# fischer-hub/panGNN

Hardware: NVIDIA B200
Metric: train_edges_per_s (higher is better)
Workload: dtype f32

## Files before the change

include/pangnn_b200.h:

```cpp
#ifndef PANGNN_B200_H
#define PANGNN_B200_H

#include <stddef.h>
#include <stdint.h>

#ifdef __cplusplus
extern "C" {
#endif

#define PANGNN_ABI_VERSION 4

#define PANGNN_OK 0
#define PANGNN_EINVAL (-1)
#define PANGNN_EWORKSPACE (-2)
#define PANGNN_ECUDA (-3)

#define PANGNN_ACT_NONE 0
#define PANGNN_ACT_ELU 1

int pangnn_abi_version(void);
const char *pangnn_last_error(void);
const char *pangnn_source_digest(void);

size_t pangnn_sort_pairs_workspace_bytes(int64_t n);
// ... 25 lines not shown
                          const float *w, const float *dis, int32_t num_nodes, int rows_are_dst,
                          float *val, void *stream);

int pangnn_gcn_aggregate(const int64_t *rowptr, const int32_t *col, const float *val, const float *x,
                         int64_t ldx, int32_t num_rows, int32_t feat, const float *bias, int act,
                         float *y, int64_t ldy, void *stream);

int pangnn_act_bwd_bias(const float *dy, const float *y, int64_t num_rows, int32_t feat, int act,
                        float *g, float *dbias , void *ws, size_t ws_bytes,
                        void *stream);
size_t pangnn_act_bwd_bias_workspace_bytes(int64_t num_rows, int32_t feat);

size_t pangnn_gemm_tn_workspace_bytes(int64_t num_rows, int32_t m, int32_t k);
int pangnn_gemm_tn(const float *a, int64_t lda, const float *b, int64_t ldb, int64_t num_rows,
                   int32_t m, int32_t k, float *c, void *ws, size_t ws_bytes, void *stream);

int pangnn_node_linear(const float *x, int64_t ldx, int64_t num_rows, int32_t k, const float *w,
                       int64_t ldw, int w_is_kn, int32_t n, const float *bias, int act, float *y,
                       int64_t ldy, void *stream);
int pangnn_node_linear_push(const float *x, int64_t ldx, int64_t num_rows, int32_t k, const float *w,
                            int64_t ldw, int w_is_kn, int32_t n, const float *bias, int act, float *y,
                            int64_t ldy, const int32_t *push_slot0, float *peer_y0, int64_t lo0, int64_t hi0,
                            const int32_t *push_slot1, float *peer_y1, int64_t lo1, int64_t hi1, void *stream);

size_t pangnn_hits_sort_unique_workspace_bytes(int64_t num_hits);
int pangnn_hits_sort_unique(const int32_t *q, const int32_t *t, const double *bits, int64_t num_hits,
                            int32_t num_nodes, int32_t *q_out, int32_t *t_out, double *bits_out,
                            uint32_t *count , void *ws, size_t ws_bytes, void *stream);
size_t pangnn_hits_normalize_workspace_bytes(int64_t num_hits);
int pangnn_hits_normalize(const int32_t *q, const int32_t *t, const double *bits, int64_t num_hits,
                          const int32_t *genome_of, const int32_t *group_of, double temp, double eps,
                          double pseudo, int drop_trivial, int32_t *src, int32_t *dst, float *w,
                          float *y, uint32_t *count , void *ws, size_t ws_bytes,
                          void *stream);

int pangnn_rows_gather_copy(const float *src, int64_t ld_src, const int32_t *idx, int64_t n, int32_t feat, float *dst,
                            int64_t ld_dst, void *stream);
int pangnn_rows_scatter_add(const float *src, int64_t ld_src, const int32_t *idx, int64_t n, int32_t feat, float *dst,
                            int64_t ld_dst, void *stream);

#define PANGNN_GRAD_REDUCE_MAX_TENSORS 32
#define PANGNN_GRAD_REDUCE_MAX_RANKS 8
int64_t pangnn_grad_bucket_floats(const int64_t *numels, int32_t count);
int pangnn_grad_push(float *const *grads, const int64_t *numels, int32_t count, float *bucket, int64_t half_floats,
                     int32_t *const *peer_signals, int32_t world, int32_t rank, int32_t *ctrl, void *stream);
int pangnn_grad_reduce(float *const *grads, const int64_t *numels, int32_t count, const float *const *peer_buckets,
// ... 123 lines not shown
```

pangnn_b200/_abi.py:

```python
import ctypes as C
import os

from . import build as _build

_c_p = C.c_void_p
_i64, _i32, _sz, _f32, _f64, _int = C.c_int64, C.c_int32, C.c_size_t, C.c_float, C.c_double, C.c_int

SIGNATURES = {
    "pangnn_abi_version": (_int, []),
    "pangnn_last_error": (C.c_char_p, []),
    "pangnn_source_digest": (C.c_char_p, []),
    "pangnn_sort_pairs_workspace_bytes": (_sz, [_i64]),
    "pangnn_sort_pairs_u64": (_int, [_c_p, _c_p, _c_p, _c_p, _i64, _int, _c_p, _sz, _c_p]),
    "pangnn_scan_workspace_bytes": (_sz, [_i64]),
    "pangnn_exclusive_scan_u32": (_int, [_c_p, _c_p, _i64, _c_p, _c_p, _sz, _c_p]),
    "pangnn_csr_build_workspace_bytes": (_sz, [_i64]),
    "pangnn_csr_build": (_int, [_c_p, _i64, _i32, _int, _c_p, _c_p, _c_p, _c_p, _sz, _c_p]),
    "pangnn_gcn_norm": (_int, [_c_p, _c_p, _c_p, _c_p, _i32, _c_p, _c_p, _c_p]),
    "pangnn_gcn_norm_apply": (_int, [_c_p, _c_p, _c_p, _c_p, _c_p, _i32, _int, _c_p, _c_p]),
    "pangnn_gcn_aggregate": (_int, [_c_p, _c_p, _c_p, _c_p, _i64, _i32, _i32, _c_p, _int, _c_p, _i64, _c_p]),
    "pangnn_act_bwd_bias": (_int, [_c_p, _c_p, _i64, _i32, _int, _c_p, _c_p, _c_p, _sz, _c_p]),
    "pangnn_act_bwd_bias_workspace_bytes": (_sz, [_i64, _i32]),
    "pangnn_gemm_tn_workspace_bytes": (_sz, [_i64, _i32, _i32]),
    "pangnn_gemm_tn": (_int, [_c_p, _i64, _c_p, _i64, _i64, _i32, _i32, _c_p, _c_p, _sz, _c_p]),
    "pangnn_node_linear": (_int, [_c_p, _i64, _i64, _i32, _c_p, _i64, _int, _i32, _c_p, _int, _c_p, _i64, _c_p]),
    "pangnn_node_linear_push": (_int, [_c_p, _i64, _i64, _i32, _c_p, _i64, _int, _i32, _c_p, _int, _c_p, _i64,
                                       _c_p, _c_p, _i64, _i64, _c_p, _c_p, _i64, _i64, _c_p]),
    "pangnn_hits_sort_unique_workspace_bytes": (_sz, [_i64]),
    "pangnn_hits_sort_unique": (_int, [_c_p, _c_p, _c_p, _i64, _i32, _c_p, _c_p, _c_p, _c_p, _c_p, _sz, _c_p]),
    "pangnn_hits_normalize_workspace_bytes": (_sz, [_i64]),
    "pangnn_hits_normalize": (_int, [_c_p, _c_p, _c_p, _i64, _c_p, _c_p, _f64, _f64, _f64, _int,
                                     _c_p, _c_p, _c_p, _c_p, _c_p, _c_p, _sz, _c_p]),
    "pangnn_rows_gather_copy": (_int, [_c_p, _i64, _c_p, _i64, _i32, _c_p, _i64, _c_p]),
    "pangnn_rows_scatter_add": (_int, [_c_p, _i64, _c_p, _i64, _i32, _c_p, _i64, _c_p]),
    "pangnn_grad_bucket_floats": (_i64, [_c_p, _i32]),
    "pangnn_grad_push": (_int, [_c_p, _c_p, _i32, _c_p, _i64, _c_p, _i32, _i32, _c_p, _c_p]),
    "pangnn_grad_reduce": (_int, [_c_p, _c_p, _i32, _c_p, _i64, _c_p, _i32, _i32, _c_p, _i64, _c_p]),
    "pangnn_edges_sorted": (_int, [_c_p, _i64, _i32, _c_p, _c_p]),
    "pangnn_csr_from_sorted": (_int, [_c_p, _i64, _i32, _c_p, _c_p, _c_p, _c_p]),
    "pangnn_csr_transpose": (_int, [_c_p, _c_p, _c_p, _i64, _i32, _c_p, _c_p, _c_p, _c_p, _sz, _c_p]),
    "pangnn_csr_merge_band": (_int, [_c_p, _c_p, _c_p, _i64, _i64, _i32, _int, _c_p, _c_p, _c_p, _c_p]),
    "pangnn_csr_spmv2": (_int, [_c_p, _c_p, _c_p, _c_p, _i32, _c_p, _c_p, _c_p]),
    "pangnn_rank1_affine_act": (_int, [_c_p, _c_p, _c_p, _c_p, _c_p, _i64, _i32, _int, _c_p, _i64, _c_p]),
    "pangnn_rank1_bwd_workspace_bytes": (_sz, [_i64, _i32]),
    "pangnn_rank1_bwd": (_int, [_c_p, _c_p, _c_p, _c_p, _i64, _i32, _int, _c_p, _c_p, _sz, _c_p]),
    "pangnn_parse_hits_tsv_workspace_bytes": (_sz, [_i64]),
    "pangnn_tsv_line_index": (_int, [_c_p, _i64, _c_p, _i64, _c_p, _c_p, _sz, _c_p]),
    "pangnn_tsv_parse_hits": (_int, [_c_p, _i64, _c_p, _i64, _i64, _i32, _c_p, _c_p, _i32, _c_p, _c_p, _c_p, _c_p]),
    "pangnn_components_init": (_int, [_c_p, _i32, _c_p]),
    "pangnn_components_round": (_int, [_c_p, _c_p, _c_p, _i64, _c_p, _i32, _c_p, _c_p]),
# ... 65 lines not shown
```

pangnn_b200/csrc/common.cuh:

```cuda
#pragma once
#include <cuda_runtime.h>
#include <stdint.h>
#include <stdio.h>

#include "../../include/pangnn_b200.h"

namespace pangnn {

constexpr int kWarp = 32;
constexpr int kNumSMs = 148;

void set_error(const char *fmt, ...);

inline int check_cuda(cudaError_t e, const char *what) {
    if (e != cudaSuccess) {
        set_error("%s: %s", what, cudaGetErrorString(e));
        return PANGNN_ECUDA;
    }
    return PANGNN_OK;
}

#define PANGNN_CHECK_LAUNCH(name)                                           \
    do {                                                                    \
        int _rc = ::pangnn::check_cuda(cudaGetLastError(), name);           \
// ... 28 lines not shown
#pragma unroll
    for (int o = 16; o > 0; o >>= 1) v += __shfl_xor_sync(0xffffffffu, v, o);
    return v;
}
__device__ __forceinline__ double warp_sum(double v) {
#pragma unroll
    for (int o = 16; o > 0; o >>= 1) v += __shfl_xor_sync(0xffffffffu, v, o);
    return v;
}
__device__ __forceinline__ double warp_max(double v) {
#pragma unroll
    for (int o = 16; o > 0; o >>= 1) v = fmax(v, __shfl_xor_sync(0xffffffffu, v, o));
    return v;
}

__device__ __forceinline__ float4 ld_stream_f4(const float *p) {
    float4 r;
    asm volatile("ld.global.nc.L1::no_allocate.v4.f32 {%0,%1,%2,%3}, [%4];"
                 : "=f"(r.x), "=f"(r.y), "=f"(r.z), "=f"(r.w)
                 : "l"(p));
    return r;
}

}
```

pangnn_b200/csrc/node_linear.cu:

```cuda
#include "common.cuh"
#include "umma.cuh"

namespace pangnn {

namespace {

constexpr int kTileM = 128;
constexpr int kKC = 32;
constexpr int kThreadsNL = 256;
constexpr int kThreadsNLAll = kThreadsNL + 32;
constexpr uint32_t kChunkA = kTileM * 16 + 16;

__device__ __forceinline__ float elu1f(float x) { return x > 0.f ? x : __expf(x) - 1.0f; }

struct NLPush {
    const int32_t *slot0, *slot1;
    float *peer0, *peer1;
    int64_t lo0, hi0, lo1, hi1;
};

template <int N, int K>
struct NLSmem {
    static constexpr uint32_t chunkB = N * 16 + 16;
    static constexpr uint32_t bytesB = (K / 4) * chunkB;
    static constexpr uint32_t bytesA = (kKC / 4) * kChunkA;
    static constexpr uint32_t ringSlot = kTileM * kKC * 4;
    static constexpr uint32_t budget = 227u * 1024u - 2048u;
    static constexpr int stages = ((int64_t)budget - (int64_t)(2 * bytesB + 4 * bytesA + 256) - 8 * 32 * (32 * 4 + 16)) / (int64_t)ringSlot >= 3 ? 2 : 1;
    static constexpr int partC = (budget - (2 * bytesB + 2 * bytesA + 256) - 8 * 32 * (32 * 4 + 16)) / ringSlot >= 3 ? 32 : 16;
    static constexpr uint32_t stageRow = partC * 4 + 16;
    static constexpr uint32_t bytesStage = 8 * 32 * stageRow;
    static constexpr uint32_t fixed = 2 * bytesB + 2 * stages * bytesA + bytesStage + 256;
    static constexpr int ringSlots = ((budget - fixed) / ringSlot) > 6 ? 6 : (int)((budget - fixed) / ringSlot);
    static constexpr uint32_t offBhi = 0, offBlo = bytesB, offA = 2 * bytesB;
    static constexpr uint32_t offStage = (offA + 2 * stages * bytesA + 127) / 128 * 128;
    static constexpr uint32_t offRing = (offStage + bytesStage + 127) / 128 * 128;
    static constexpr uint32_t total = offRing + ringSlots * ringSlot + 64;
    static constexpr int tmemCols = 4 * N;
    static_assert(ringSlots >= 2, "ring too small");
};

__device__ __forceinline__ void cp_async16(uint32_t dst_smem, const void *src) {
    asm volatile("cp.async.cg.shared.global [%0], [%1], 16;" :: "r"(dst_smem), "l"(src) : "memory");
}
__device__ __forceinline__ void cp_async_commit() { asm volatile("cp.async.commit_group;" ::: "memory"); }
template <int NPENDING>
__device__ __forceinline__ void cp_async_wait() { asm volatile("cp.async.wait_group %0;" :: "n"(NPENDING) : "memory"); }

template <int N, int K>
__global__ void __launch_bounds__(kThreadsNLAll, 1)
node_linear_kernel(const float *__restrict__ x, int64_t ldx, int64_t M, const float *__restrict__ w,
                   int64_t ldw, int w_is_kn, const float *__restrict__ bias, int act,
                   float *__restrict__ y, int64_t ldy, const NLPush push) {
    using S = NLSmem<N, K>;
    extern __shared__ __align__(128) uint8_t smem[];
    __shared__ __align__(8) uint64_t bar_stage[2], bar_ready[2], bar_full[2], bar_dfree[2];
    __shared__ uint32_t tmem_base_s;
    const int tid = threadIdx.x, warp = tid >> 5, lane = tid & 31;
    const uint32_t sbase = umma::smem_u32(smem);
    constexpr int NCH = K / kKC;
    constexpr int RS = S::ringSlots;

    if (warp == 0) umma::tmem_alloc(&tmem_base_s, S::tmemCols);
    if (tid == 32) {
        umma::mbar_init(&bar_stage[0], 1);
        umma::mbar_init(&bar_stage[1], 1);
        umma::mbar_init(&bar_full[0], 1);
        umma::mbar_init(&bar_full[1], 1);
        umma::mbar_init(&bar_ready[0], kThreadsNL);
        umma::mbar_init(&bar_ready[1], kThreadsNL);
        umma::mbar_init(&bar_dfree[0], kThreadsNL);
        umma::mbar_init(&bar_dfree[1], kThreadsNL);
        umma::fence_mbar_init();
    }
    for (int idx = tid; idx < N * K; idx += kThreadsNLAll) {
        int n, k;
// ... 12 lines not shown
    const uint32_t tmem_d = tmem_base_s;

    const int64_t num_tiles = (M + kTileM - 1) / kTileM;
    const int64_t my_tiles = blockIdx.x < num_tiles ? (num_tiles - blockIdx.x + gridDim.x - 1) / gridDim.x : 0;
    const int64_t n_items = my_tiles * NCH;
    const int f = tid & 7, rb = tid >> 3;
    constexpr uint32_t idesc = umma::idesc_tf32(kTileM, N, false, false);

    auto issue_item = [&](int64_t it) {
        if (it < n_items) {
            const int64_t tile = blockIdx.x + (it / NCH) * gridDim.x;
            const int c = (int)(it % NCH);
            const uint32_t slot = sbase + S::offRing + (uint32_t)(it % RS) * S::ringSlot;
#pragma unroll
            for (int i = 0; i < 4; ++i) {
                const int r = rb + 32 * i;
                const int64_t row = tile * kTileM + r;
                if (row < M) cp_async16(slot + (uint32_t)r * 128 + (uint32_t)f * 16, x + row * ldx + c * kKC + f * 4);
            }
        }
        cp_async_commit();
    };

    auto epilogue = [&](int64_t t_local) {
        const int64_t tile = blockIdx.x + t_local * gridDim.x;
        const int buf = (int)(t_local & 1);
        umma::mbar_wait(&bar_full[buf], (uint32_t)((t_local >> 1) & 1));
        umma::fence_after_sync();
        const int q = warp & 3, h = warp >> 2;
        constexpr int COLS = N / 2;
        constexpr int PC = S::partC;
        uint8_t *stg = smem + S::offStage + (uint32_t)warp * 32 * S::stageRow;
        const int64_t row0 = tile * kTileM + q * 32;
#pragma unroll
        for (int part = 0; part < COLS / PC; ++part) {
            const int c0 = h * COLS + part * PC;
            float v[PC], vs[PC];
            const uint32_t ta = tmem_d + (uint32_t)(buf * 2 * N) + ((uint32_t)(q * 32) << 16) + (uint32_t)c0;
            umma::tmem_ld<PC>(ta, v);
            umma::tmem_ld<PC>(ta + N, vs);
#pragma unroll
            for (int j = 0; j < PC; ++j) v[j] += vs[j];
#pragma unroll
            for (int j = 0; j < PC; j += 4) {
                float4 o = make_float4(v[j], v[j + 1], v[j + 2], v[j + 3]);
                if (bias) {
                    const float4 b = __ldg(reinterpret_cast<const float4 *>(bias + c0 + j));
                    o.x += b.x; o.y += b.y; o.z += b.z; o.w += b.w;
                }
                if (act == PANGNN_ACT_ELU) { o.x = elu1f(o.x); o.y = elu1f(o.y); o.z = elu1f(o.z); o.w = elu1f(o.w); }
                *reinterpret_cast<float4 *>(stg + (uint32_t)lane * S::stageRow + j * 4) = o;
            }
            __syncwarp();
            constexpr int LPR = PC / 4;
#pragma unroll
            for (int r0 = 0; r0 < 32; r0 += 32 / LPR) {
                const int r = r0 + lane / LPR, fl = lane % LPR;
                const float4 o = *reinterpret_cast<const float4 *>(stg + (uint32_t)r * S::stageRow + fl * 16);
                if (row0 + r < M) {
                    *reinterpret_cast<float4 *>(y + (row0 + r) * ldy + c0 + fl * 4) = o;
                    const int64_t gr = row0 + r;
                    if (push.slot0 && gr >= push.lo0 && gr < push.hi0) {
                        const int32_t ps = __ldg(push.slot0 + gr);
                        if (ps >= 0) *reinterpret_cast<float4 *>(push.peer0 + (int64_t)ps * ldy + c0 + fl * 4) = o;
                    }
                    if (push.slot1 && gr >= push.lo1 && gr < push.hi1) {
                        const int32_t ps = __ldg(push.slot1 + gr);
                        if (ps >= 0) *reinterpret_cast<float4 *>(push.peer1 + (int64_t)ps * ldy + c0 + fl * 4) = o;
                    }
                }
            }
            __syncwarp();
        }
        umma::fence_before_sync();
    };

    constexpr int ST = S::stages;
    if (warp == kThreadsNL / 32) {
#pragma unroll 1
        for (int64_t it = 0; it < n_items; ++it) {
            const int64_t t_local = it / NCH;
            const int c = (int)(it % NCH);
// ... 37 lines not shown
            if (it >= ST) umma::mbar_wait(&bar_stage[st], (uint32_t)(((it - ST) / ST) & 1));
            const uint32_t offAhi = S::offA + (uint32_t)st * 2 * S::bytesA, offAlo = offAhi + S::bytesA;
#pragma unroll
            for (int i = 0; i < 4; ++i) {
                float4 hi, lo;
                umma::split4(raw[i], hi, lo);
                const uint32_t off = (uint32_t)f * kChunkA + (uint32_t)(rb + 32 * i) * 16;
                *reinterpret_cast<float4 *>(smem + offAhi + off) = hi;
                *reinterpret_cast<float4 *>(smem + offAlo + off) = lo;
            }
            umma::fence_async_smem();
            umma::mbar_arrive(&bar_ready[st]);
            if (c == 0 && t_local > 0) {
                epilogue(t_local - 1);
                umma::mbar_arrive(&bar_dfree[(t_local - 1) & 1]);
            }
        }
        if (my_tiles > 0) epilogue(my_tiles - 1);
        cp_async_wait<0>();
    }
    umma::fence_before_sync();
    __syncthreads();
    if (warp == 0) umma::tmem_dealloc(tmem_d, S::tmemCols);
}

template <int N, int K>
int launch_node_linear(const float *x, int64_t ldx, int64_t M, const float *w, int64_t ldw, int w_is_kn,
                       const float *bias, int act, float *y, int64_t ldy, const NLPush &push, cudaStream_t st) {
    using S = NLSmem<N, K>;
    static bool attr_set = false;
    if (!attr_set) {
        int rc = check_cuda(cudaFuncSetAttribute(node_linear_kernel<N, K>, cudaFuncAttributeMaxDynamicSharedMemorySize,
                                                 (int)S::total), "cudaFuncSetAttribute(node_linear)");
        if (rc) return rc;
        attr_set = true;
    }
    const int64_t tiles = (M + kTileM - 1) / kTileM;
    const unsigned grid = (unsigned)(tiles < kNumSMs ? tiles : kNumSMs);
    node_linear_kernel<N, K><<<grid, kThreadsNLAll, S::total, st>>>(x, ldx, M, w, ldw, w_is_kn, bias, act, y, ldy, push);
    PANGNN_CHECK_LAUNCH("node_linear");
    return PANGNN_OK;
}

}
}

using namespace pangnn;

static int node_linear_dispatch(const float *x, int64_t ldx, int64_t num_rows, int32_t k, const float *w, int64_t ldw,
                                int w_is_kn, int32_t n, const float *bias, int act, float *y, int64_t ldy,
                                const NLPush &push, void *stream) {
    PANGNN_REQUIRE(num_rows >= 0, "negative row count");
    if (num_rows == 0) return PANGNN_OK;
    PANGNN_REQUIRE(x && w && y, "null pointer");
    PANGNN_REQUIRE((n == 64 || n == 128) && (k == 64 || k == 128), "n and k must be 64 or 128");
    PANGNN_REQUIRE(ldx % 4 == 0 && ldy % 4 == 0 && ldx >= k && ldy >= n, "bad row stride");
    PANGNN_REQUIRE(ldw >= (w_is_kn ? n : k), "bad weight stride");
    PANGNN_REQUIRE((uintptr_t)x % 16 == 0 && (uintptr_t)y % 16 == 0 && (!bias || (uintptr_t)bias % 16 == 0),
                   "pointers must be 16-byte aligned");
    PANGNN_REQUIRE((!push.slot0 || (push.peer0 && (uintptr_t)push.peer0 % 16 == 0)) &&
                       (!push.slot1 || (push.peer1 && (uintptr_t)push.peer1 % 16 == 0)), "bad push target");
    cudaStream_t st = (cudaStream_t)stream;
    if (n == 64 && k == 64) return launch_node_linear<64, 64>(x, ldx, num_rows, w, ldw, w_is_kn, bias, act, y, ldy, push, st);
    if (n == 128 && k == 64) return launch_node_linear<128, 64>(x, ldx, num_rows, w, ldw, w_is_kn, bias, act, y, ldy, push, st);
    if (n == 64 && k == 128) return launch_node_linear<64, 128>(x, ldx, num_rows, w, ldw, w_is_kn, bias, act, y, ldy, push, st);
    return launch_node_linear<128, 128>(x, ldx, num_rows, w, ldw, w_is_kn, bias, act, y, ldy, push, st);
}

extern "C" int pangnn_node_linear(const float *x, int64_t ldx, int64_t num_rows, int32_t k, const float *w,
                                  int64_t ldw, int w_is_kn, int32_t n, const float *bias, int act, float *y,
                                  int64_t ldy, void *stream) {
    return node_linear_dispatch(x, ldx, num_rows, k, w, ldw, w_is_kn, n, bias, act, y, ldy, NLPush{nullptr, nullptr, nullptr, nullptr, 0, 0, 0, 0},
                                stream);
}

extern "C" int pangnn_node_linear_push(const float *x, int64_t ldx, int64_t num_rows, int32_t k, const float *w,
                                       int64_t ldw, int w_is_kn, int32_t n, const float *bias, int act, float *y,
                                       int64_t ldy, const int32_t *push_slot0, float *peer_y0, int64_t lo0, int64_t hi0,
                                       const int32_t *push_slot1, float *peer_y1, int64_t lo1, int64_t hi1,
                                       void *stream) {
    return node_linear_dispatch(x, ldx, num_rows, k, w, ldw, w_is_kn, n, bias, act, y, ldy,
                                NLPush{push_slot0, push_slot1, peer_y0, peer_y1, lo0, hi0, lo1, hi1}, stream);
}
```

pangnn_b200/csrc/rank1.cu:

```cuda
#include "common.cuh"

namespace pangnn {

int reduce_partials(const float *partial, int64_t nblocks, int32_t width, int32_t stride, float *out,
                    cudaStream_t st);

__global__ void __launch_bounds__(256)
csr_spmv2_kernel(const int64_t *__restrict__ rowptr, const int32_t *__restrict__ col, const float *__restrict__ val,
                 const float *__restrict__ x, int32_t N, float *__restrict__ ax, float *__restrict__ a1) {
    const int lane = threadIdx.x & 31;
    const int64_t row = ((int64_t)blockIdx.x * blockDim.x + threadIdx.x) >> 5;
    if (row >= N) return;
    const int64_t b = rowptr[row], e = rowptr[row + 1];
    double sx = 0.0, s1 = 0.0;
    for (int64_t i = b + lane; i < e; i += 32) {
        const double v = (double)val[i];
        s1 += v;
        sx += x ? v * (double)x[col[i]] : v;
    }
    sx = warp_sum(sx);
    s1 = warp_sum(s1);
    if (lane == 0) {
        ax[row] = (float)sx;
        a1[row] = (float)s1;
    }
}

__device__ __forceinline__ float act_apply(float x, int act) {
    return (act == PANGNN_ACT_ELU && x <= 0.f) ? expm1f(x) : x;
}

__global__ void __launch_bounds__(256)
rank1_affine_act_kernel(const float *__restrict__ a, const float *__restrict__ c, const float *__restrict__ u,
                        const float *__restrict__ v, const float *__restrict__ bias, int64_t num_rows, int32_t fq,
                        int act, float *__restrict__ y, int64_t ldy) {
    const int64_t i = (int64_t)blockIdx.x * blockDim.x + threadIdx.x;
    if (i >= num_rows * fq) return;
    const int64_t r = i / fq;
    const int t = (int)(i % fq);
    const float ar = a[r], cr = c[r];
    const float4 uu = __ldg(reinterpret_cast<const float4 *>(u) + t), vv = __ldg(reinterpret_cast<const float4 *>(v) + t);
    float4 bb = make_float4(0.f, 0.f, 0.f, 0.f);
    if (bias) bb = __ldg(reinterpret_cast<const float4 *>(bias) + t);
    float4 o;
    o.x = act_apply(fmaf(ar, uu.x, fmaf(cr, vv.x, bb.x)), act);
    o.y = act_apply(fmaf(ar, uu.y, fmaf(cr, vv.y, bb.y)), act);
    o.z = act_apply(fmaf(ar, uu.z, fmaf(cr, vv.z, bb.z)), act);
    o.w = act_apply(fmaf(ar, uu.w, fmaf(cr, vv.w, bb.w)), act);
    reinterpret_cast<float4 *>(y + r * ldy)[t] = o;
}

constexpr int kR1RowsPerChunk = 64;
constexpr int kR1MaxBlocks = kNumSMs * 8;

__global__ void __launch_bounds__(256)
rank1_bwd_kernel(const float *__restrict__ dy, const float *__restrict__ yv, const float *__restrict__ a,
                 const float *__restrict__ c, int64_t num_rows, int32_t feat, int act, float *__restrict__ partial) {
    extern __shared__ float4 red[];
    const int fq = feat / 4;
    const int tx = threadIdx.x % fq, ty = threadIdx.x / fq;
    const int TY = blockDim.x / fq;
    const int64_t nchunks = (num_rows + kR1RowsPerChunk - 1) / kR1RowsPerChunk;
    float4 s0 = make_float4(0.f, 0.f, 0.f, 0.f), s1 = s0, s2 = s0;
    if (ty < TY) {
        for (int64_t chunk = blockIdx.x; chunk < nchunks; chunk += gridDim.x) {
            const int64_t r0 = chunk * kR1RowsPerChunk;
            const int64_t r1 = min(r0 + (int64_t)kR1RowsPerChunk, num_rows);
            for (int64_t r = r0 + ty; r < r1; r += TY) {
                float4 d = ld_stream_f4(dy + r * feat + tx * 4);
                if (act == PANGNN_ACT_ELU) {
                    const float4 o = ld_stream_f4(yv + r * feat + tx * 4);
// ... 91 lines not shown
```

pangnn_b200/gnn.py:

```python
import math

import torch
from torch import nn

from . import ops
from .setup import args


_SIDE_STREAMS = {}

OPERATOR_LAYER = {"kind": "function"}


def set_operator_layer(kind):
    if kind not in ("function", "library"):
        raise ValueError("operator layer is 'function' or 'library'")
    OPERATOR_LAYER["kind"] = kind


def _side_stream(device):
    key = torch.device(device).index
    if key not in _SIDE_STREAMS:
        _SIDE_STREAMS[key] = torch.cuda.Stream(device=device)
    return _SIDE_STREAMS[key]
# ... 28 lines not shown
        super().__init__()
        self.device = device
        node_embedding_dim, hidden_dim = dims
        if categorical_nodes:
            num = dataset if isinstance(dataset, int) else int(getattr(dataset, "num_genes", 0) or len(dataset.x))
            self.embedding = nn.Embedding(num, node_embedding_dim)
        else:
            self.embedding = nn.Linear(1, node_embedding_dim)
        self.conv_in = GCNConv(node_embedding_dim, hidden_dim, add_self_loops=False)
        self.conv_hidden = GCNConv(hidden_dim, hidden_dim, add_self_loops=False)
        self.conv_out = GCNConv(hidden_dim, node_embedding_dim, add_self_loops=False)
        self.linear_out = nn.Linear(hidden_dim, node_embedding_dim)
        self.activation_fct = nn.ELU()
        self.mlp = nn.Sequential(
            nn.Linear(node_embedding_dim * 2 + (1 if args.skip_connections else 0), node_embedding_dim),
            nn.ReLU(),
            nn.Linear(node_embedding_dim, node_embedding_dim),
            nn.ReLU(),
            nn.Linear(node_embedding_dim, 1))
        self.epoch = 0
        self._categorical = bool(categorical_nodes)
        self.fuse_embedding = True

    def embed(self, graph):
        ELU = ops.ACT_ELU
        if (not self._categorical and graph.x.dim() == 2 and graph.x.size(1) == 1 and self.fuse_embedding
                and OPERATOR_LAYER["kind"] == "function"
                and self.conv_in.out_channels % 4 == 0 and self.conv_in.out_channels <= 256):
            ei = graph.union_edge_index if args.union_edge_weights else graph.edge_index
            emb, cin = self.embedding, self.conv_in
            nodes = ops.embed_conv(graph.x, emb.weight, emb.bias, cin.lin.weight, cin.bias, ei, graph.edge_attr, ELU)
            return self._embed_tail(graph, nodes)
        if self._categorical:
            idx = graph.x if graph.x.dtype == torch.long else (
                graph.node_id if hasattr(graph, "node_id") else
                torch.arange(graph.x.size(0), device=graph.x.device))
            node_embeddings = self.embedding(idx)
        elif graph.x.dim() == 2 and graph.x.size(1) == 1:
            node_embeddings = torch.addcmul(self.embedding.bias, graph.x, self.embedding.weight.t())
        else:
            node_embeddings = self.embedding(graph.x)
        ei = graph.union_edge_index if args.union_edge_weights else graph.edge_index
        nodes = self.conv_in(node_embeddings, ei, graph.edge_attr, _act=ELU)
        return self._embed_tail(graph, nodes)

    def _embed_tail(self, graph, nodes):
        ELU = ops.ACT_ELU
        if args.union_edge_weights:
            for _ in range(max(args.neighbours - 2, 1)):
                nodes = self.conv_hidden(nodes, graph.union_edge_index, graph.edge_attr, _act=ELU)
            nodes = self.conv_out(nodes, graph.union_edge_index, None, _act=ELU)
# ... 81 lines not shown
                    gs = ops.graph_struct(graph.edge_index, n)
                    gs.src, gs.endpoints32
                    gs.built_on(side, main)
                graph.edge_index.record_stream(side)
            wait(*[k for k in ("edge_attr", "x", "y") if k in ready])
            return graph
        wait("edge_index")
        gs = ops.graph_struct(graph.edge_index, n)
        gs.src, gs.endpoints32
        if not args.base_model:
            if getattr(graph, "neighbour_edge_index", None) is None:
                graph.neighbour_edge_index = ops.neighbour_band(n, args.neighbours, graph.edge_index.device)
            wait("neighbour_edge_index")
            ops.graph_struct(graph.neighbour_edge_index, n).src
        wait()
        return graph

    def forward_loss(self, graph, pos_weight):
        if not self._use_fused_mlp_flag():
            logits = self.forward(graph)
            loss = torch.nn.functional.binary_cross_entropy_with_logits(
                logits, graph.y, pos_weight=torch.as_tensor(float(pos_weight), device=logits.device))
            return loss, logits.detach()
        nodes = self.embed(graph)
        gs = ops.graph_struct(graph.edge_index, nodes.size(0))
        m = self.mlp
        if OPERATOR_LAYER["kind"] == "library":
            from . import torch_ops
            return torch_ops.score_edges_bce(nodes, m[0].weight, m[0].bias, m[2].weight, m[2].bias, m[4].weight,
                                             m[4].bias, graph.edge_index, self._skip(graph), graph.y, float(pos_weight))
        return ops.EdgeScoreBCEFn.apply(
            nodes, m[0].weight, m[0].bias, m[2].weight, m[2].bias, m[4].weight, m[4].bias,
            gs, self._skip(graph), graph.y, float(pos_weight))

    def _use_fused_mlp_flag(self):
        return args.decoder == "mlp" and self.mlp[2].weight.size(0) == ops.SCORER_D

    def decode(self, z, edge_index):
        return ops.edge_pair_score(z, ops.graph_struct(edge_index, z.size(0)), 1)

    def cosine_sim(self, z, edge_index):
        return ops.edge_pair_score(z, ops.graph_struct(edge_index, z.size(0)), 0)
```

pangnn_b200/ops.py:

```python
import ctypes as C
from collections import OrderedDict, namedtuple

import torch

from . import _abi

ACT_NONE, ACT_ELU = 0, 1
SCORER_D = 64
NGRADS = 64 * 64 + 64 + 64 + 1 + 64 + 64

LAUNCHES = {"count": 0}


def _p(t):
    return C.c_void_p(t.data_ptr()) if t is not None else C.c_void_p(0)


def _stream():
    return C.c_void_p(torch.cuda.current_stream().cuda_stream)


def _need_cuda(*ts):
    for t in ts:
        if t is not None and not t.is_cuda:
# ... 265 lines not shown
        if act == ACT_ELU:
            torch.nn.functional.elu_(y)
        if out is not None:
            out.copy_(y)
            return out
        return y
    lib = _abi.load()
    M = x.size(0)
    if out is None:
        out = torch.empty(M, n, dtype=torch.float32, device=x.device)
    if push is None:
        _abi.check(lib.pangnn_node_linear(_p(x), x.stride(0), M, k, _p(w), w.stride(0), 1 if w_is_kn else 0, n,
                                          _p(bias), act, _p(out), out.stride(0), _stream()), "node_linear")
    else:
        (s0, p0, lo0, hi0), (s1, p1, lo1, hi1) = (list(push) + [(None, None, 0, 0), (None, None, 0, 0)])[:2]
        for pt in (p0, p1):
            if pt is not None and pt.stride(0) != out.stride(0):
                raise _abi.PangnnError("peer buffers must have the row stride of the output")
        _abi.check(lib.pangnn_node_linear_push(_p(x), x.stride(0), M, k, _p(w), w.stride(0), 1 if w_is_kn else 0, n,
                                               _p(bias), act, _p(out), out.stride(0), _p(s0), _p(p0), lo0, hi0,
                                               _p(s1), _p(p1), lo1, hi1, _stream()), "node_linear_push")
    LAUNCHES["count"] += 1
    return out


class GraphStruct:

    def __init__(self, edge_index, num_nodes):
        self.edge_index = edge_index
        self.num_nodes = num_nodes
        self.num_edges = edge_index.size(1)
        self._src = None
        if self.num_edges > SMALL_CSR_EDGES and edge_index.dtype == torch.int64 and edge_index.dim() == 2:
            self._src = csr_from_sorted(edge_index, num_nodes)
        self._dst = csr_transpose(self._src) if self._src is not None else csr_build(edge_index, num_nodes, by_dst=True)
        self._ends = None
        self._norm = OrderedDict()
        self._ready = None

    def built_on(self, stream, user_stream):
        ev = torch.cuda.Event()
        ev.record(stream)
        self._ready = ev
        for t in (self._dst, self._src):
            if t is not None:
                for a in (t.rowptr, t.col, t.perm):
# ... 285 lines not shown
    args, E = _scorer_operands(pq, w1c, b1, w2, b2, w3, b3, gs, skip)
    dev = pq.device
    if da1 is None:
        da1 = torch.empty(E, SCORER_D, dtype=torch.float32, device=dev)
    if grads is None:
        grads = torch.empty(NGRADS, dtype=torch.float32, device=dev)
    if ws is None:
        ws = _ws(lib.pangnn_edge_score_workspace_bytes(E), dev)
    dlogits = None if dlogits is None else dlogits.contiguous()
    y = None if y is None else y.contiguous()
    _abi.check(lib.pangnn_edge_score_bwd(*map(_p, args), E, _p(dlogits), _p(y), float(pos_weight), float(scale),
                                         _p(da1), _p(grads), _p(logits), _p(loss_sum), _p(ws), ws.numel(), _stream()),
               "edge_score_bwd")
    LAUNCHES["count"] += 2 + (loss_sum is not None)
    return da1, grads


def _scorer_common(h, w1, skip):
    if h.size(1) != SCORER_D or w1.size(0) != SCORER_D:
        raise _abi.PangnnError("the fused edge scorer is built for --node_dim 64")
    return split_w1(w1, skip is not None)


def _unpack_scorer_grads(grads, da1, gs, h, wcat, skip, need_h, scale=None):
    D = SCORER_D
    N = h.size(0)
    dpq = torch.empty(N, 2 * D, dtype=torch.float32, device=h.device)
    segment_sum_edges(gs.src, da1, N, dpq[:, :D])
    segment_sum_edges(gs.dst, da1, N, dpq[:, D:])
    dwcat = gemm_tn(dpq, h)
    if scale is not None:
        grads, dwcat, wcat = grads * scale, dwcat * scale, wcat * scale
    g = scorer_grads(grads)
    dw1 = torch.cat((dwcat[:D], dwcat[D:]) + ((g.dw1c.unsqueeze(1),) if skip is not None else ()), dim=1)
    dh = node_linear(dpq, wcat, w_is_kn=True) if need_h else None
    return dh, dw1, g.db1, g.dW2, g.db2, g.dw3, g.db3


class EdgeScoreFn(torch.autograd.Function):

    @staticmethod
    def forward(ctx, h, w1, b1, w2, b2, w3, b3, gs, skip):
        wcat, w1c = _scorer_common(h, w1, skip)
        pq = node_linear(h, wcat)
        logits = edge_score_pq_fwd(pq, w1c, b1, w2, b2, w3, b3, gs, skip)
        ctx.gs, ctx.skip = gs, skip
        ctx.save_for_backward(h, w1, b1, w2, b2, w3, b3, pq)
        return logits

    @staticmethod
    def backward(ctx, dlogits):
        h, w1, b1, w2, b2, w3, b3, pq = ctx.saved_tensors
        gs, skip = ctx.gs, ctx.skip
        wcat, w1c = _scorer_common(h, w1, skip)
        da1, grads = edge_score_train(pq, w1c, b1, w2, b2, w3, b3, gs, skip, dlogits=dlogits)
        return _unpack_scorer_grads(grads, da1, gs, h, wcat, skip, ctx.needs_input_grad[0]) + (None, None)


class EdgeScoreBCEFn(torch.autograd.Function):

    @staticmethod
    def forward(ctx, h, w1, b1, w2, b2, w3, b3, gs, skip, y, pos_weight):
        wcat, w1c = _scorer_common(h, w1, skip)
        E = gs.num_edges
        pq = node_linear(h, wcat)
        logits = torch.empty(E, dtype=torch.float32, device=h.device)
        loss_sum = torch.zeros(1, dtype=torch.float64, device=h.device)
        da1, grads = edge_score_train(pq, w1c, b1, w2, b2, w3, b3, gs, skip, y=y, pos_weight=pos_weight,
                                      scale=1.0 / max(E, 1), logits=logits, loss_sum=loss_sum)
        ctx.gs, ctx.skip = gs, skip
        ctx.save_for_backward(h, wcat, da1, grads)
        ctx.mark_non_differentiable(logits)
        loss = (loss_sum / max(E, 1)).float().squeeze(0)
        return loss, logits

    @staticmethod
    def backward(ctx, dloss, _dlogits):
        h, wcat, da1, grads = ctx.saved_tensors
        out = _unpack_scorer_grads(grads, da1, ctx.gs, h, wcat, ctx.skip, ctx.needs_input_grad[0],
                                   scale=dloss)
        return out + (None, None, None, None)


class EdgePairScoreFn(torch.autograd.Function):

    @staticmethod
    def forward(ctx, h, gs, mode):
        lib = _abi.load()
        src, dst = gs.endpoints32
        h = h.contiguous()
        out = torch.empty(gs.num_edges, dtype=torch.float32, device=h.device)
        _abi.check(lib.pangnn_edge_pair_score(_p(h), h.stride(0), h.size(1), _p(src), _p(dst),
                                              gs.num_edges, mode, _p(out), _stream()), "edge_pair_score")
        LAUNCHES["count"] += 1
        ctx.gs, ctx.mode = gs, mode
        ctx.save_for_backward(h, out)
        return out

    @staticmethod
    def backward(ctx, dz):
        lib = _abi.load()
        h, out = ctx.saved_tensors
        gs = ctx.gs
        N, F = h.shape
# ... 663 lines not shown
```

Before: 890.2 million.

## Fuse whole embed-GCN-scorer training step into one autograd function with fused backward epilogues

Adds a node_linear backward mode whose tensor-core epilogue applies the ELU derivative and accumulates per-column bias-gradient sums, plus a rank-2 mode that recomputes the first-layer activation from a, c, u and v instead of storing it. These feed a new autograd function that runs the embedding, the GCN layers and the scorer BCE as a single forward and backward. The goal is to remove separate activation-backward, bias-reduction and elementwise kernels and the autograd overhead between layers. In exchange the node_linear kernel gains epilogue register pressure and a per-block partial-sum reduction, and the fused path only applies to specific shapes and flags.

```diff
diff --git a/include/pangnn_b200.h b/include/pangnn_b200.h
--- a/include/pangnn_b200.h
+++ b/include/pangnn_b200.h
@@ -71,6 +71,13 @@
                             int64_t ldw, int w_is_kn, int32_t n, const float *bias, int act, float *y,
                             int64_t ldy, const int32_t *push_slot0, float *peer_y0, int64_t lo0, int64_t hi0,
                             const int32_t *push_slot1, float *peer_y1, int64_t lo1, int64_t hi1, void *stream);
+#define PANGNN_NL_ACT_GRAD 1
+#define PANGNN_NL_RANK2 2
+size_t pangnn_node_linear_bwd_workspace_bytes(int64_t num_rows, int32_t n);
+int pangnn_node_linear_bwd(const float *x, int64_t ldx, int64_t num_rows, int32_t k, const float *w, int64_t ldw,
+                           int32_t n, int mode, const float *y, int64_t ldy, const float *a, const float *c,
+                           const float *u, const float *v, const float *bias, float *g, int64_t ldg, float *sums,
+                           void *ws, size_t ws_bytes, void *stream);
 
 size_t pangnn_hits_sort_unique_workspace_bytes(int64_t num_hits);
 int pangnn_hits_sort_unique(const int32_t *q, const int32_t *t, const double *bits, int64_t num_hits,
diff --git a/pangnn_b200/_abi.py b/pangnn_b200/_abi.py
--- a/pangnn_b200/_abi.py
+++ b/pangnn_b200/_abi.py
@@ -26,6 +26,9 @@
     "pangnn_node_linear": (_int, [_c_p, _i64, _i64, _i32, _c_p, _i64, _int, _i32, _c_p, _int, _c_p, _i64, _c_p]),
     "pangnn_node_linear_push": (_int, [_c_p, _i64, _i64, _i32, _c_p, _i64, _int, _i32, _c_p, _int, _c_p, _i64,
                                        _c_p, _c_p, _i64, _i64, _c_p, _c_p, _i64, _i64, _c_p]),
+    "pangnn_node_linear_bwd_workspace_bytes": (_sz, [_i64, _i32]),
+    "pangnn_node_linear_bwd": (_int, [_c_p, _i64, _i64, _i32, _c_p, _i64, _i32, _int, _c_p, _i64, _c_p, _c_p, _c_p,
+                                      _c_p, _c_p, _c_p, _i64, _c_p, _c_p, _sz, _c_p]),
     "pangnn_hits_sort_unique_workspace_bytes": (_sz, [_i64]),
     "pangnn_hits_sort_unique": (_int, [_c_p, _c_p, _c_p, _i64, _i32, _c_p, _c_p, _c_p, _c_p, _c_p, _sz, _c_p]),
     "pangnn_hits_normalize_workspace_bytes": (_sz, [_i64]),
diff --git a/pangnn_b200/csrc/common.cuh b/pangnn_b200/csrc/common.cuh
--- a/pangnn_b200/csrc/common.cuh
+++ b/pangnn_b200/csrc/common.cuh
@@ -74,4 +74,9 @@
     return r;
 }
 
+__device__ __forceinline__ float rank2_act(float a, float c, float u, float v, float b, int act) {
+    const float x = fmaf(a, u, fmaf(c, v, b));
+    return (act == PANGNN_ACT_ELU && x <= 0.f) ? expm1f(x) : x;
 }
+
+}
diff --git a/pangnn_b200/csrc/node_linear.cu b/pangnn_b200/csrc/node_linear.cu
--- a/pangnn_b200/csrc/node_linear.cu
+++ b/pangnn_b200/csrc/node_linear.cu
@@ -2,6 +2,9 @@
 #include "umma.cuh"
 
 namespace pangnn {
+
+int reduce_partials(const float *partial, int64_t nblocks, int32_t width, int32_t stride, float *out,
+                    cudaStream_t st);
 
 namespace {
 
@@ -17,6 +20,14 @@
     const int32_t *slot0, *slot1;
     float *peer0, *peer1;
     int64_t lo0, hi0, lo1, hi1;
+};
+
+enum { kEpiStore = 0, kEpiActGrad = 1, kEpiRank2 = 2 };
+struct NLBwd {
+    const float *yv;
+    int64_t ldyv;
+    const float *a, *c, *u, *v, *bias;
+    float *partial;
 };
 
 template <int N, int K>
@@ -47,11 +58,11 @@
 template <int NPENDING>
 __device__ __forceinline__ void cp_async_wait() { asm volatile("cp.async.wait_group %0;" :: "n"(NPENDING) : "memory"); }
 
-template <int N, int K>
+template <int N, int K, int EPI>
 __global__ void __launch_bounds__(kThreadsNLAll, 1)
 node_linear_kernel(const float *__restrict__ x, int64_t ldx, int64_t M, const float *__restrict__ w,
                    int64_t ldw, int w_is_kn, const float *__restrict__ bias, int act,
-                   float *__restrict__ y, int64_t ldy, const NLPush push) {
+                   float *__restrict__ y, int64_t ldy, const NLPush push, const NLBwd bw) {
     using S = NLSmem<N, K>;
     extern __shared__ __align__(128) uint8_t smem[];
     __shared__ __align__(8) uint64_t bar_stage[2], bar_ready[2], bar_full[2], bar_dfree[2];
@@ -110,6 +121,14 @@
         cp_async_commit();
     };
 
+    constexpr int NS = EPI == kEpiRank2 ? 3 : 1;
+    constexpr int NPART = (N / 2) / S::partC;
+    float csum[NS][NPART][4];
+#pragma unroll
+    for (int s = 0; s < NS; ++s)
+#pragma unroll
+        for (int p = 0; p < NPART; ++p) csum[s][p][0] = csum[s][p][1] = csum[s][p][2] = csum[s][p][3] = 0.f;
+
     auto epilogue = [&](int64_t t_local) {
         const int64_t tile = blockIdx.x + t_local * gridDim.x;
         const int buf = (int)(t_local & 1);
@@ -144,8 +163,40 @@
 #pragma unroll
             for (int r0 = 0; r0 < 32; r0 += 32 / LPR) {
                 const int r = r0 + lane / LPR, fl = lane % LPR;
-                const float4 o = *reinterpret_cast<const float4 *>(stg + (uint32_t)r * S::stageRow + fl * 16);
-                if (row0 + r < M) {
+                float4 o = *reinterpret_cast<const float4 *>(stg + (uint32_t)r * S::stageRow + fl * 16);
+                if (EPI == kEpiActGrad && row0 + r < M) {
+                    const float4 yy = ld_stream_f4(bw.yv + (row0 + r) * bw.ldyv + c0 + fl * 4);
+                    o.x *= yy.x > 0.f ? 1.f : yy.x + 1.f;
+                    o.y *= yy.y > 0.f ? 1.f : yy.y + 1.f;
+                    o.z *= yy.z > 0.f ? 1.f : yy.z + 1.f;
+                    o.w *= yy.w > 0.f ? 1.f : yy.w + 1.f;
+                    *reinterpret_cast<float4 *>(y + (row0 + r) * ldy + c0 + fl * 4) = o;
+                    float *cs = csum[0][part];
+                    cs[0] += o.x; cs[1] += o.y; cs[2] += o.z; cs[3] += o.w;
+                } else if (EPI == kEpiRank2 && row0 + r < M) {
+                    const int col = c0 + fl * 4;
+                    const float ar = __ldg(bw.a + row0 + r), cr = __ldg(bw.c + row0 + r);
+                    const float4 uu = __ldg(reinterpret_cast<const float4 *>(bw.u + col));
+                    const float4 vv = __ldg(reinterpret_cast<const float4 *>(bw.v + col));
+                    const float4 bb = bw.bias ? __ldg(reinterpret_cast<const float4 *>(bw.bias + col))
+                                              : make_float4(0.f, 0.f, 0.f, 0.f);
+                    float4 y0;
+                    y0.x = rank2_act(ar, cr, uu.x, vv.x, bb.x, PANGNN_ACT_ELU);
+                    y0.y = rank2_act(ar, cr, uu.y, vv.y, bb.y, PANGNN_ACT_ELU);
+                    y0.z = rank2_act(ar, cr, uu.z, vv.z, bb.z, PANGNN_ACT_ELU);
+                    y0.w = rank2_act(ar, cr, uu.w, vv.w, bb.w, PANGNN_ACT_ELU);
+                    o.x *= y0.x > 0.f ? 1.f : y0.x + 1.f;
+                    o.y *= y0.y > 0.f ? 1.f : y0.y + 1.f;
+                    o.z *= y0.z > 0.f ? 1.f : y0.z + 1.f;
+                    o.w *= y0.w > 0.f ? 1.f : y0.w + 1.f;
+                    const float ov[4] = {o.x, o.y, o.z, o.w};
+#pragma unroll
+                    for (int e = 0; e < 4; ++e) {
+                        csum[0][part][e] += ov[e];
+                        csum[NS > 1 ? 1 : 0][part][e] = fmaf(ar, ov[e], csum[NS > 1 ? 1 : 0][part][e]);
+                        csum[NS > 2 ? 2 : 0][part][e] = fmaf(cr, ov[e], csum[NS > 2 ? 2 : 0][part][e]);
+                    }
+                } else if (EPI == kEpiStore && row0 + r < M) {
                     *reinterpret_cast<float4 *>(y + (row0 + r) * ldy + c0 + fl * 4) = o;
                     const int64_t gr = row0 + r;
                     if (push.slot0 && gr >= push.lo0 && gr < push.hi0) {
@@ -229,25 +280,64 @@
     umma::fence_before_sync();
     __syncthreads();
     if (warp == 0) umma::tmem_dealloc(tmem_d, S::tmemCols);
-}
-
-template <int N, int K>
+    if constexpr (EPI != kEpiStore) {
+        constexpr int LPR = S::partC / 4;
+        float *red = reinterpret_cast<float *>(smem + S::offStage);
+        static_assert(4 * NS * N * 4 <= S::bytesStage, "staging area too small for the column sums");
+        if (warp < kThreadsNL / 32) {
+            const int q = warp & 3, h = warp >> 2;
+#pragma unroll
+            for (int s = 0; s < NS; ++s)
+#pragma unroll
+                for (int p = 0; p < NPART; ++p)
+#pragma unroll
+                    for (int e = 0; e < 4; ++e) {
+                        float t = csum[s][p][e];
+#pragma unroll
+                        for (int o = 16; o >= LPR; o >>= 1) t += __shfl_xor_sync(0xffffffffu, t, o);
+                        if (lane < LPR) red[(q * NS + s) * N + h * (N / 2) + p * S::partC + lane * 4 + e] = t;
+                    }
+        }
+        __syncthreads();
+        for (int i = tid; i < NS * N; i += kThreadsNLAll)
+            bw.partial[(int64_t)blockIdx.x * NS * N + i] = ((red[i] + red[NS * N + i]) + red[2 * NS * N + i]) + red[3 * NS * N + i];
+    }
+}
+
+int64_t node_linear_grid(int64_t M) {
+    const int64_t tiles = (M + kTileM - 1) / kTileM;
+    return tiles < kNumSMs ? tiles : kNumSMs;
+}
+
+template <int N, int K, int EPI>
 int launch_node_linear(const float *x, int64_t ldx, int64_t M, const float *w, int64_t ldw, int w_is_kn,
-                       const float *bias, int act, float *y, int64_t ldy, const NLPush &push, cudaStream_t st) {
+                       const float *bias, int act, float *y, int64_t ldy, const NLPush &push, const NLBwd &bw,
+                       cudaStream_t st) {
     using S = NLSmem<N, K>;
     static bool attr_set = false;
     if (!attr_set) {
-        int rc = check_cuda(cudaFuncSetAttribute(node_linear_kernel<N, K>, cudaFuncAttributeMaxDynamicSharedMemorySize,
+        int rc = check_cuda(cudaFuncSetAttribute(node_linear_kernel<N, K, EPI>, cudaFuncAttributeMaxDynamicSharedMemorySize,
                                                  (int)S::total), "cudaFuncSetAttribute(node_linear)");
         if (rc) return rc;
         attr_set = true;
     }
-    const int64_t tiles = (M + kTileM - 1) / kTileM;
-    const unsigned grid = (unsigned)(tiles < kNumSMs ? tiles : kNumSMs);
-    node_linear_kernel<N, K><<<grid, kThreadsNLAll, S::total, st>>>(x, ldx, M, w, ldw, w_is_kn, bias, act, y, ldy, push);
+    const unsigned grid = (unsigned)node_linear_grid(M);
+    node_linear_kernel<N, K, EPI><<<grid, kThreadsNLAll, S::total, st>>>(x, ldx, M, w, ldw, w_is_kn, bias, act, y, ldy,
+                                                                          push, bw);
     PANGNN_CHECK_LAUNCH("node_linear");
     return PANGNN_OK;
 }
+
+template <int EPI>
+int launch_node_linear_nk(int n, int k, const float *x, int64_t ldx, int64_t M, const float *w, int64_t ldw,
+                          int w_is_kn, const float *bias, int act, float *y, int64_t ldy, const NLPush &push,
+                          const NLBwd &bw, cudaStream_t st) {
+    if (n == 64 && k == 64) return launch_node_linear<64, 64, EPI>(x, ldx, M, w, ldw, w_is_kn, bias, act, y, ldy, push, bw, st);
+    if (n == 128 && k == 64) return launch_node_linear<128, 64, EPI>(x, ldx, M, w, ldw, w_is_kn, bias, act, y, ldy, push, bw, st);
+    if (n == 64 && k == 128) return launch_node_linear<64, 128, EPI>(x, ldx, M, w, ldw, w_is_kn, bias, act, y, ldy, push, bw, st);
+    return launch_node_linear<128, 128, EPI>(x, ldx, M, w, ldw, w_is_kn, bias, act, y, ldy, push, bw, st);
+}
+
 
 }
 }
@@ -267,11 +357,9 @@
                    "pointers must be 16-byte aligned");
     PANGNN_REQUIRE((!push.slot0 || (push.peer0 && (uintptr_t)push.peer0 % 16 == 0)) &&
                        (!push.slot1 || (push.peer1 && (uintptr_t)push.peer1 % 16 == 0)), "bad push target");
-    cudaStream_t st = (cudaStream_t)stream;
-    if (n == 64 && k == 64) return launch_node_linear<64, 64>(x, ldx, num_rows, w, ldw, w_is_kn, bias, act, y, ldy, push, st);
-    if (n == 128 && k == 64) return launch_node_linear<128, 64>(x, ldx, num_rows, w, ldw, w_is_kn, bias, act, y, ldy, push, st);
-    if (n == 64 && k == 128) return launch_node_linear<64, 128>(x, ldx, num_rows, w, ldw, w_is_kn, bias, act, y, ldy, push, st);
-    return launch_node_linear<128, 128>(x, ldx, num_rows, w, ldw, w_is_kn, bias, act, y, ldy, push, st);
+    const NLBwd none{nullptr, 0, nullptr, nullptr, nullptr, nullptr, nullptr, nullptr};
+    return launch_node_linear_nk<kEpiStore>(n, k, x, ldx, num_rows, w, ldw, w_is_kn, bias, act, y, ldy, push, none,
+                                            (cudaStream_t)stream);
 }
 
 extern "C" int pangnn_node_linear(const float *x, int64_t ldx, int64_t num_rows, int32_t k, const float *w,
@@ -289,3 +377,48 @@
     return node_linear_dispatch(x, ldx, num_rows, k, w, ldw, w_is_kn, n, bias, act, y, ldy,
                                 NLPush{push_slot0, push_slot1, peer_y0, peer_y1, lo0, hi0, lo1, hi1}, stream);
 }
+
+extern "C" size_t pangnn_node_linear_bwd_workspace_bytes(int64_t num_rows, int32_t n) {
+    const int64_t grid = node_linear_grid(num_rows < 1 ? 1 : num_rows);
+    return (size_t)grid * 3 * (n > 0 ? n : 0) * sizeof(float) + 256;
+}
+
+extern "C" int pangnn_node_linear_bwd(const float *x, int64_t ldx, int64_t num_rows, int32_t k, const float *w,
+                                      int64_t ldw, int32_t n, int mode, const float *y, int64_t ldy, const float *a,
+                                      const float *c, const float *u, const float *v, const float *bias, float *g,
+                                      int64_t ldg, float *sums, void *ws, size_t ws_bytes, void *stream) {
+    PANGNN_REQUIRE(mode == PANGNN_NL_ACT_GRAD || mode == PANGNN_NL_RANK2, "unknown mode");
+    PANGNN_REQUIRE(num_rows >= 0, "negative row count");
+    PANGNN_REQUIRE((n == 64 || n == 128) && (k == 64 || k == 128), "n and k must be 64 or 128");
+    PANGNN_REQUIRE(sums && ws, "null pointer");
+    if (ws_bytes < pangnn_node_linear_bwd_workspace_bytes(num_rows, n)) {
+        set_error("node_linear_bwd: workspace too small");
+        return PANGNN_EWORKSPACE;
+    }
+    cudaStream_t st = (cudaStream_t)stream;
+    const int ns = mode == PANGNN_NL_RANK2 ? 3 : 1;
+    if (num_rows == 0) return check_cuda(cudaMemsetAsync(sums, 0, (size_t)ns * n * sizeof(float), st), "memset");
+    PANGNN_REQUIRE(x && w, "null pointer");
+    PANGNN_REQUIRE(ldx % 4 == 0 && ldx >= k && ldw >= n, "bad row stride");
+    PANGNN_REQUIRE((uintptr_t)x % 16 == 0, "pointers must be 16-byte aligned");
+    const NLPush no_push{nullptr, nullptr, nullptr, nullptr, 0, 0, 0, 0};
+    float *partial = static_cast<float *>(ws);
+    int rc;
+    if (mode == PANGNN_NL_ACT_GRAD) {
+        PANGNN_REQUIRE(y && g, "null pointer");
+        PANGNN_REQUIRE(ldy % 4 == 0 && ldg % 4 == 0 && ldy >= n && ldg >= n, "bad row stride");
+        PANGNN_REQUIRE((uintptr_t)y % 16 == 0 && (uintptr_t)g % 16 == 0, "pointers must be 16-byte aligned");
+        const NLBwd bw{y, ldy, nullptr, nullptr, nullptr, nullptr, nullptr, partial};
+        rc = launch_node_linear_nk<kEpiActGrad>(n, k, x, ldx, num_rows, w, ldw, 1, nullptr, PANGNN_ACT_NONE, g, ldg,
+                                                no_push, bw, st);
+    } else {
+        PANGNN_REQUIRE(a && c && u && v && !g, "rank-2 mode: a, c, u, v required, no output");
+        PANGNN_REQUIRE((uintptr_t)u % 16 == 0 && (uintptr_t)v % 16 == 0 && (!bias || (uintptr_t)bias % 16 == 0),
+                       "pointers must be 16-byte aligned");
+        const NLBwd bw{nullptr, 0, a, c, u, v, bias, partial};
+        rc = launch_node_linear_nk<kEpiRank2>(n, k, x, ldx, num_rows, w, ldw, 1, nullptr, PANGNN_ACT_NONE, nullptr, 0,
+                                              no_push, bw, st);
+    }
+    if (rc) return rc;
+    return reduce_partials(partial, node_linear_grid(num_rows), ns * n, ns * n, sums, st);
+}
diff --git a/pangnn_b200/csrc/rank1.cu b/pangnn_b200/csrc/rank1.cu
--- a/pangnn_b200/csrc/rank1.cu
+++ b/pangnn_b200/csrc/rank1.cu
@@ -26,10 +26,6 @@
     }
 }
 
-__device__ __forceinline__ float act_apply(float x, int act) {
-    return (act == PANGNN_ACT_ELU && x <= 0.f) ? expm1f(x) : x;
-}
-
 __global__ void __launch_bounds__(256)
 rank1_affine_act_kernel(const float *__restrict__ a, const float *__restrict__ c, const float *__restrict__ u,
                         const float *__restrict__ v, const float *__restrict__ bias, int64_t num_rows, int32_t fq,
@@ -43,10 +39,10 @@
     float4 bb = make_float4(0.f, 0.f, 0.f, 0.f);
     if (bias) bb = __ldg(reinterpret_cast<const float4 *>(bias) + t);
     float4 o;
-    o.x = act_apply(fmaf(ar, uu.x, fmaf(cr, vv.x, bb.x)), act);
-    o.y = act_apply(fmaf(ar, uu.y, fmaf(cr, vv.y, bb.y)), act);
-    o.z = act_apply(fmaf(ar, uu.z, fmaf(cr, vv.z, bb.z)), act);
-    o.w = act_apply(fmaf(ar, uu.w, fmaf(cr, vv.w, bb.w)), act);
+    o.x = rank2_act(ar, cr, uu.x, vv.x, bb.x, act);
+    o.y = rank2_act(ar, cr, uu.y, vv.y, bb.y, act);
+    o.z = rank2_act(ar, cr, uu.z, vv.z, bb.z, act);
+    o.w = rank2_act(ar, cr, uu.w, vv.w, bb.w, act);
     reinterpret_cast<float4 *>(y + r * ldy)[t] = o;
 }
 
diff --git a/pangnn_b200/gnn.py b/pangnn_b200/gnn.py
--- a/pangnn_b200/gnn.py
+++ b/pangnn_b200/gnn.py
@@ -74,11 +74,14 @@
         self._categorical = bool(categorical_nodes)
         self.fuse_embedding = True
 
+    def _rank2_first_layer(self, graph):
+        return (not self._categorical and graph.x.dim() == 2 and graph.x.size(1) == 1 and self.fuse_embedding
+                and OPERATOR_LAYER["kind"] == "function"
+                and self.conv_in.out_channels % 4 == 0 and self.conv_in.out_channels <= 256)
+
     def embed(self, graph):
         ELU = ops.ACT_ELU
-        if (not self._categorical and graph.x.dim() == 2 and graph.x.size(1) == 1 and self.fuse_embedding
-                and OPERATOR_LAYER["kind"] == "function"
-                and self.conv_in.out_channels % 4 == 0 and self.conv_in.out_channels <= 256):
+        if self._rank2_first_layer(graph):
             ei = graph.union_edge_index if args.union_edge_weights else graph.edge_index
             emb, cin = self.embedding, self.conv_in
             nodes = ops.embed_conv(graph.x, emb.weight, emb.bias, cin.lin.weight, cin.bias, ei, graph.edge_attr, ELU)
@@ -206,6 +209,8 @@
             loss = torch.nn.functional.binary_cross_entropy_with_logits(
                 logits, graph.y, pos_weight=torch.as_tensor(float(pos_weight), device=logits.device))
             return loss, logits.detach()
+        if self._fused_step(graph):
+            return self._forward_loss_fused(graph, pos_weight)
         nodes = self.embed(graph)
         gs = ops.graph_struct(graph.edge_index, nodes.size(0))
         m = self.mlp
@@ -217,6 +222,28 @@
             nodes, m[0].weight, m[0].bias, m[2].weight, m[2].bias, m[4].weight, m[4].bias,
             gs, self._skip(graph), graph.y, float(pos_weight))
 
+    def _fused_step(self, graph):
+        return (self._rank2_first_layer(graph) and self.conv_in.out_channels in (64, 128)
+                and self.conv_out.out_channels == ops.SCORER_D and (args.union_edge_weights or not args.base_model)
+                and not graph.x.requires_grad)
+
+    def _forward_loss_fused(self, graph, pos_weight):
+        n = graph.x.size(0)
+        if args.union_edge_weights:
+            ue = ops.graph_struct(graph.union_edge_index, n)
+            first = ue
+            convs = [(0, ue, graph.edge_attr)] * max(args.neighbours - 2, 1) + [(1, ue, None)]
+        else:
+            first = ops.graph_struct(graph.edge_index, n)
+            convs = [(1, ops.graph_struct(graph.neighbour_edge_index, n), None)]
+        a, c = ops._rank1_cached(first, graph.edge_attr, graph.x)
+        gs = ops.graph_struct(graph.edge_index, n)
+        emb, cin, chid, cout, m = self.embedding, self.conv_in, self.conv_hidden, self.conv_out, self.mlp
+        return ops.EmbedScoreBCEFn.apply(
+            a, c, emb.weight, emb.bias, cin.lin.weight, cin.bias, chid.lin.weight, chid.bias, cout.lin.weight,
+            cout.bias, m[0].weight, m[0].bias, m[2].weight, m[2].bias, m[4].weight, m[4].bias, convs,
+            (gs, self._skip(graph), graph.y, float(pos_weight)))
+
     def _use_fused_mlp_flag(self):
         return args.decoder == "mlp" and self.mlp[2].weight.size(0) == ops.SCORER_D
 
diff --git a/pangnn_b200/ops.py b/pangnn_b200/ops.py
--- a/pangnn_b200/ops.py
+++ b/pangnn_b200/ops.py
@@ -311,6 +311,40 @@
                                                _p(s1), _p(p1), lo1, hi1, _stream()), "node_linear_push")
     LAUNCHES["count"] += 1
     return out
+
+
+def _node_linear_bwd(x, w, mode, y=None, rank2=None):
+    lib = _abi.load()
+    _need_cuda(x, w)
+    k, n = w.shape
+    if not _tc_shape(x, n, k) or x.size(1) != k or w.stride(1) != 1:
+        raise _abi.PangnnError("node_linear_bwd needs the tensor-core shapes (n, k in {64, 128}, aligned rows)")
+    M = x.size(0)
+    ns = 3 if mode == 2 else 1
+    sums = torch.empty(ns, n, dtype=torch.float32, device=x.device)
+    ws = _ws(lib.pangnn_node_linear_bwd_workspace_bytes(M, n), x.device)
+    g = None
+    if mode == 1:
+        y = _rows16(y)
+        g = torch.empty(M, n, dtype=torch.float32, device=x.device)
+        a = c = u = v = b = None
+    else:
+        a, c, u, v, b = rank2
+    _abi.check(lib.pangnn_node_linear_bwd(_p(x), x.stride(0), M, k, _p(w), w.stride(0), n, mode, _p(y),
+                                          0 if y is None else y.stride(0), _p(a), _p(c), _p(u), _p(v), _p(b), _p(g),
+                                          0 if g is None else g.stride(0), _p(sums), _p(ws), ws.numel(), _stream()),
+               "node_linear_bwd")
+    LAUNCHES["count"] += 2
+    return g, sums
+
+
+def node_linear_act_grad(x, w, y):
+    g, sums = _node_linear_bwd(x, w, 1, y=y)
+    return g, sums[0]
+
+
+def node_linear_rank2(x, w, a, c, u, v, bias):
+    return _node_linear_bwd(x, w, 2, rank2=(a, c, u, v, bias))[1]
 
 
 class GraphStruct:
@@ -642,7 +676,7 @@
     return split_w1(w1, skip is not None)
 
 
-def _unpack_scorer_grads(grads, da1, gs, h, wcat, skip, need_h, scale=None):
+def _scorer_node_grads(grads, da1, gs, h, wcat, skip, scale=None):
     D = SCORER_D
     N = h.size(0)
     dpq = torch.empty(N, 2 * D, dtype=torch.float32, device=h.device)
@@ -653,8 +687,13 @@
         grads, dwcat, wcat = grads * scale, dwcat * scale, wcat * scale
     g = scorer_grads(grads)
     dw1 = torch.cat((dwcat[:D], dwcat[D:]) + ((g.dw1c.unsqueeze(1),) if skip is not None else ()), dim=1)
+    return dpq, wcat, (dw1, g.db1, g.dW2, g.db2, g.dw3, g.db3)
+
+
+def _unpack_scorer_grads(grads, da1, gs, h, wcat, skip, need_h, scale=None):
+    dpq, wcat, wgrads = _scorer_node_grads(grads, da1, gs, h, wcat, skip, scale)
     dh = node_linear(dpq, wcat, w_is_kn=True) if need_h else None
-    return dh, dw1, g.db1, g.dW2, g.db2, g.dw3, g.db3
+    return (dh,) + wgrads
 
 
 class EdgeScoreFn(torch.autograd.Function):
@@ -700,6 +739,65 @@
         out = _unpack_scorer_grads(grads, da1, ctx.gs, h, wcat, ctx.skip, ctx.needs_input_grad[0],
                                    scale=dloss)
         return out + (None, None, None, None)
+
+
+class EmbedScoreBCEFn(torch.autograd.Function):
+
+    @staticmethod
+    def forward(ctx, a, c, w_e, b_e, w_in, b_in, w_hid, b_hid, w_out, b_out, w1, b1, w2, b2, w3, b3, convs, scored):
+        lib = _abi.load()
+        N, F = a.numel(), w_in.size(0)
+        w_e1 = w_e.reshape(-1)
+        u, v = torch.mv(w_in, w_e1), torch.mv(w_in, b_e)
+        y = torch.empty(N, F, dtype=torch.float32, device=a.device)
+        _abi.check(lib.pangnn_rank1_affine_act(_p(a), _p(c), _p(u), _p(v), _p(b_in), N, F, ACT_ELU, _p(y),
+                                               y.stride(0), _stream()), "rank1_affine_act")
+        LAUNCHES["count"] += 1
+        layers = ((w_hid, b_hid), (w_out, b_out))
+        ys = [y]
+        for li, gs, ew in convs:
+            weight, bias = layers[li]
+            ent = gs.norm(ew, need_src=False)
+            h = node_linear(ys[-1], weight)
+            ys.append(aggregate(gs, ent, h, True, bias, ACT_ELU))
+        gs, skip, lab, pos_weight = scored
+        wcat, w1c = _scorer_common(ys[-1], w1, skip)
+        E = gs.num_edges
+        pq = node_linear(ys[-1], wcat)
+        logits = torch.empty(E, dtype=torch.float32, device=a.device)
+        loss_sum = torch.zeros(1, dtype=torch.float64, device=a.device)
+        da1, grads = edge_score_train(pq, w1c, b1, w2, b2, w3, b3, gs, skip, y=lab, pos_weight=pos_weight,
+                                      scale=1.0 / max(E, 1), logits=logits, loss_sum=loss_sum)
+        ctx.convs, ctx.gs, ctx.skip = convs, gs, skip
+        ctx.save_for_backward(a, c, u, v, w_e1, b_e, w_in, b_in, w_hid, w_out, w1, da1, grads, *ys)
+        ctx.mark_non_differentiable(logits)
+        return (loss_sum / max(E, 1)).float().squeeze(0), logits
+
+    @staticmethod
+    def backward(ctx, dloss, _dlogits):
+        a, c, u, v, w_e1, b_e, w_in, b_in, w_hid, w_out, w1, da1, grads, *ys = ctx.saved_tensors
+        wcat, _ = _scorer_common(ys[-1], w1, ctx.skip)
+        dpq, wcat, scorer = _scorer_node_grads(grads, da1, ctx.gs, ys[-1], wcat, ctx.skip, scale=dloss)
+        g, db = node_linear_act_grad(dpq, wcat, ys[-1])
+        dw, dbias = [None, None], [None, None]
+        sums = None
+        for i in range(len(ctx.convs) - 1, -1, -1):
+            li, gs, ew = ctx.convs[i]
+            weight = (w_hid, w_out)[li]
+            dh = aggregate(gs, gs.norm(ew, need_src=True), g, False)
+            dwi = gemm_tn(dh, ys[i])
+            dw[li] = dwi if dw[li] is None else dw[li] + dwi
+            dbias[li] = db if dbias[li] is None else dbias[li] + db
+            if i > 0:
+                g, db = node_linear_act_grad(dh, weight, ys[i])
+            else:
+                sums = node_linear_rank2(dh, weight, a, c, u, v, b_in)
+        db_in, du, dv = sums[0], sums[1], sums[2]
+        dW_in = torch.addr(torch.outer(du, w_e1), dv, b_e)
+        dw_e = torch.mv(w_in.t(), du).unsqueeze(1)
+        db_e = torch.mv(w_in.t(), dv)
+        return ((None, None, dw_e, db_e, dW_in, db_in, dw[0], dbias[0], dw[1], dbias[1]) + scorer
+                + (None, None))
 
 
 class EdgePairScoreFn(torch.autograd.Function):
```

Measured after the change: 861.4 million (median of 6 runs). 3.2% lower.
